# tencent-ailab/V-Express

Measured on AMD Instinct MI355X. Metric: decoded frames/sec at 512x512, 25 DDIM steps, higher is better.
Workload: dtype bf16; 1 GPU; 512x512, 16 frames (1 window(s) of 16, overlap 4), 25 DDIM steps, CFG 3.5, random-init UNet3D + ReferenceNet banks + sd-vae-ft-mse decode; frames=16, windows=1, parallelism=window x CFG-half units over 1 GPU(s)

## Files before the change

### v-express_amd/csrc/vx_attn.hip

```cpp
#include "vx_common.h"
#include <stdio.h>
#include "../../include/vexpress_hip.h"

#include <stdlib.h>

#include <type_traits>

namespace {

struct AttnParams {
  const bf16_t* q; int ldq;
  const bf16_t* k; int ldk;
  const bf16_t* vt; int vt_pitch;
  bf16_t* out; int ldo;
  int batch, heads, n_q, n_kv, d, q_per_kv;
  float c;
  const float* kmax;
};

__device__ __forceinline__ int k_lds_off(int slab, int key, int grp) {
  return slab * 4096 + key * 64 + ((grp ^ ((0 - (key >> 2)) & 3)) << 4);
}
__device__ __forceinline__ int v_lds_off(int row, int chunk) { return row * 128 + ((chunk ^ ((row >> 1) & 7)) << 4); }

// ... 658 lines not shown
    for (int half = 0; half < 2; ++half) {
      bf16_t e0 = 0, e1 = 0, e2 = 0, e3 = 0;
      if (half < FT && dcol < 32 * KK) {
        int fr0 = 16 * half + 4 * g;
        e0 = vsm[wave][fr0 + 0][dcol]; e1 = vsm[wave][fr0 + 1][dcol];
        e2 = vsm[wave][fr0 + 2][dcol]; e3 = vsm[wave][fr0 + 3][dcol];
      }
      w[2 * half + 0] = (uint32_t)e0 | ((uint32_t)e1 << 16);
      w[2 * half + 1] = (uint32_t)e2 | ((uint32_t)e3 << 16);
    }
    uint4 vf = make_uint4(w[0], w[1], w[2], w[3]);
#pragma unroll
    for (int qt = 0; qt < FT; ++qt) {
      f32x4_t acc = mfma16(vf, pb[qt], f32x4_t{0.f, 0.f, 0.f, 0.f});
      int fr = 16 * qt + i;
      int dc = 16 * dt + 4 * g;
      if (live && fr < p.f && dc < p.d) {
        uint2 st;
        st.x = pack_bf16x2(acc[0] * inv_l[qt], acc[1] * inv_l[qt]);
        st.y = pack_bf16x2(acc[2] * inv_l[qt], acc[3] * inv_l[qt]);
        *reinterpret_cast<uint2*>(p.out + ((size_t)(bb * p.f + fr) * p.hw + pix) * p.ldo + h * p.d + dc) = st;
      }
    }
  }
}

template <int KK, int DT>
int launch_temporal(const TemporalParams& p, hipStream_t stream) {
  long waves = (long)p.b * p.hw * p.heads;
  static int wpb_env = -1;
  if (wpb_env < 0) {
    const char* e = getenv("VX_TEMPORAL_WPB");
    wpb_env = e ? atoi(e) : 0;
  }
  const bool wide = wpb_env ? wpb_env == 8 : (p.heads % 8) == 0;
  static char sym[4][56];
  auto name = [&](int slot, int ft, int wpb) {
    if (!sym[slot][0]) snprintf(sym[slot], sizeof(sym[slot]), "temporal_attn_kernel<%d, %d, %d, %d>", KK, DT, ft, wpb);
    g_vx_last_kernel = sym[slot];
  };
  if (wide && (p.heads % 8) == 0 && KK * (p.f <= 16 ? 1 : 2) <= 6) {
    dim3 grid((unsigned)((waves + 7) / 8));
    name(p.f <= 16 ? 0 : 1, p.f <= 16 ? 1 : 2, 8);
    if (p.f <= 16) hipLaunchKernelGGL((temporal_attn_kernel<KK, DT, 1, 8>), grid, dim3(512), 0, stream, p);
    else hipLaunchKernelGGL((temporal_attn_kernel<KK, DT, 2, 8>), grid, dim3(512), 0, stream, p);
    return vx_check_launch("vx_temporal_attention");
  }
  dim3 grid((unsigned)((waves + 3) / 4));
  name(p.f <= 16 ? 2 : 3, p.f <= 16 ? 1 : 2, 4);
  if (p.f <= 16) hipLaunchKernelGGL((temporal_attn_kernel<KK, DT, 1, 4>), grid, dim3(256), 0, stream, p);
  else hipLaunchKernelGGL((temporal_attn_kernel<KK, DT, 2, 4>), grid, dim3(256), 0, stream, p);
  return vx_check_launch("vx_temporal_attention");
}

constexpr int SKV_MAX = 16;

__global__ __launch_bounds__(256) void small_kv_attn_kernel(const bf16_t* __restrict__ q, int ldq,
                                                            const bf16_t* __restrict__ kv, int ldkv, int v_off,
                                                            bf16_t* __restrict__ out, int ldo, int n_q, int n_kv,
                                                            int heads, int d, float c) {
  extern __shared__ __attribute__((aligned(16))) char smem[];
  bf16_t* kvs = reinterpret_cast<bf16_t*>(smem);
  const int C = heads * d;
  const int b = blockIdx.y;
  const int tid = threadIdx.x;
  const int cch = C >> 3;
  for (int idx = tid; idx < n_kv * 2 * cch; idx += 256) {
    int j = idx / (2 * cch), rem = idx % (2 * cch);
    int which = rem / cch, ch = (rem % cch) * 8;
    const bf16_t* src = kv + ((size_t)b * n_kv + j) * ldkv + (which ? v_off : 0) + ch;
    *reinterpret_cast<uint4*>(kvs + ((size_t)(j * 2 + which)) * C + ch) = *reinterpret_cast<const uint4*>(src);
  }
  __syncthreads();
  const long item = (long)blockIdx.x * 256 + tid;
  if (item >= (long)n_q * heads) return;
  const int h = (int)(item % heads);
  const int tok = (int)(item / heads);
  const bf16_t* qp = q + ((size_t)b * n_q + tok) * ldq + h * d;
  float sc[SKV_MAX];
#pragma unroll
  for (int j = 0; j < SKV_MAX; ++j) sc[j] = 0.f;
  for (int ch = 0; ch < d; ch += 8) {
    float qv[8];
    unpack_bf16x8(*reinterpret_cast<const uint4*>(qp + ch), qv);
#pragma unroll
    for (int j = 0; j < SKV_MAX; ++j) {
      if (j < n_kv) {
        float kvv[8];
        unpack_bf16x8(*reinterpret_cast<const uint4*>(kvs + (size_t)(j * 2) * C + h * d + ch), kvv);
#pragma unroll
        for (int e = 0; e < 8; ++e) sc[j] = fmaf(qv[e], kvv[e], sc[j]);
      }
    }
  }
  float mx = -INFINITY;
#pragma unroll
  for (int j = 0; j < SKV_MAX; ++j)
    if (j < n_kv) mx = fmaxf(mx, sc[j]);
  float den = 0.f;
#pragma unroll
  for (int j = 0; j < SKV_MAX; ++j) {
    float pv = (j < n_kv) ? __builtin_amdgcn_exp2f((sc[j] - mx) * c) : 0.f;
    sc[j] = pv;
    den += pv;
  }
  const float inv = 1.0f / den;
  bf16_t* op = out + ((size_t)b * n_q + tok) * ldo + h * d;
  for (int ch = 0; ch < d; ch += 8) {
    float acc[8] = {0.f, 0.f, 0.f, 0.f, 0.f, 0.f, 0.f, 0.f};
#pragma unroll
    for (int j = 0; j < SKV_MAX; ++j) {
      if (j < n_kv) {
        float vv[8];
        unpack_bf16x8(*reinterpret_cast<const uint4*>(kvs + (size_t)(j * 2 + 1) * C + h * d + ch), vv);
#pragma unroll
        for (int e = 0; e < 8; ++e) acc[e] = fmaf(sc[j], vv[e], acc[e]);
      }
    }
#pragma unroll
    for (int e = 0; e < 8; ++e) acc[e] *= inv;
    *reinterpret_cast<uint4*>(op + ch) = pack_bf16x8(acc);
  }
}

__global__ __launch_bounds__(256) void key_norm_max_kernel(const bf16_t* __restrict__ k, int ldk, int heads, int n_kv,
                                                           int d, float* __restrict__ out) {
  __shared__ float red[256];
  const int bh = blockIdx.x, b = bh / heads, h = bh - b * heads;
  const bf16_t* base = k + (size_t)b * n_kv * ldk + h * d;
  const int chunks = d >> 3;
  float best = 0.f;
  for (int key = threadIdx.x; key < n_kv; key += 256) {
    const bf16_t* row = base + (size_t)key * ldk;
    float ss = 0.f;
    for (int c = 0; c < chunks; ++c) {
      float f[8];
      unpack_bf16x8(*reinterpret_cast<const uint4*>(row + 8 * c), f);
#pragma unroll
      for (int e = 0; e < 8; ++e) ss = fmaf(f[e], f[e], ss);
    }
    best = fmaxf(best, ss);
  }
  red[threadIdx.x] = best;
  __syncthreads();
  for (int s = 128; s > 0; s >>= 1) {
    if ((int)threadIdx.x < s) red[threadIdx.x] = fmaxf(red[threadIdx.x], red[threadIdx.x + s]);
    __syncthreads();
  }
  if (threadIdx.x == 0) out[bh] = sqrtf(red[0]);
}

constexpr int KNM8_KEYS = 256;
__global__ __launch_bounds__(256) void key_norm_max8_kernel(const bf16_t* __restrict__ k, int ldk, int n_kv, int d,
                                                            float* __restrict__ out) {
  __shared__ float red[4][8];
  const int b = blockIdx.y, key0 = blockIdx.x * KNM8_KEYS;
  const int lane = threadIdx.x & 63, wave = threadIdx.x >> 6, h = lane & 7;
  const bf16_t* base = k + (size_t)b * n_kv * ldk + h * d;
  const int chunks = d >> 3;
  float best = 0.f;
  for (int kk = wave * 8 + (lane >> 3); kk < KNM8_KEYS; kk += 32) {
    const int key = min(key0 + kk, n_kv - 1);
    const bf16_t* row = base + (size_t)key * ldk;
    float ss = 0.f;
    for (int c = 0; c < chunks; ++c) {
      float f[8];
      unpack_bf16x8(*reinterpret_cast<const uint4*>(row + 8 * c), f);
#pragma unroll
      for (int e = 0; e < 8; ++e) ss = fmaf(f[e], f[e], ss);
    }
    best = fmaxf(best, ss);
  }
  best = fmaxf(best, __shfl_xor(best, 8, 64));
  best = fmaxf(best, __shfl_xor(best, 16, 64));
  best = fmaxf(best, __shfl_xor(best, 32, 64));
  if (lane < 8) red[wave][lane] = best;
  __syncthreads();
  if (threadIdx.x < 8) {
    const float m = fmaxf(fmaxf(red[0][threadIdx.x], red[1][threadIdx.x]), fmaxf(red[2][threadIdx.x], red[3][threadIdx.x]));
    atomicMax(reinterpret_cast<unsigned int*>(out) + b * 8 + threadIdx.x, __float_as_uint(sqrtf(m)));
  }
}

int attention_impl(const void* q, int ldq, const void* k, int ldk, const void* vt, int vt_pitch, void* out, int ldo,
                   int batch, int heads, int n_q, int n_kv, int head_dim, int q_per_kv, float scale,
                   const float* key_norm_max, hipStream_t stream);

}

int vx_attn3_variant();
int vx_attn3_launch(const void* q, int ldq, const void* k, int ldk, const void* vt, int vt_pitch, void* out, int ldo,
                    int batch, int heads, int n_q, int n_kv, int q_per_kv, float c, const float* kmax,
                    hipStream_t stream);

extern "C" int vx_key_norm_max(const void* k, int ldk, int kv_batches, int heads, int n_kv, int head_dim, float* out,
                               void* stream) {
  VX_REQUIRE(k && out, "vx_key_norm_max: null pointer");
  VX_REQUIRE(kv_batches > 0 && heads > 0 && n_kv > 0 && head_dim > 0 && (head_dim % 8) == 0 && (ldk % 8) == 0,
             "vx_key_norm_max: bad sizes (head_dim=%d ldk=%d)", head_dim, ldk);
  static int v8 = -1;
  if (v8 < 0) {
    const char* e = getenv("VX_KNM8");
    v8 = !(e && atoi(e) == 0);
  }
  if (v8 && heads == 8 && n_kv >= 2 * KNM8_KEYS && kv_batches <= 65535) {
    if (hipMemsetAsync(out, 0, (size_t)kv_batches * heads * sizeof(float), (hipStream_t)stream) != hipSuccess) {
      vx_set_error("vx_key_norm_max: hipMemsetAsync failed");
      return VX_ERR_HIP;
    }
    hipLaunchKernelGGL(key_norm_max8_kernel, dim3((n_kv + KNM8_KEYS - 1) / KNM8_KEYS, kv_batches), dim3(256), 0,
                       (hipStream_t)stream, (const bf16_t*)k, ldk, n_kv, head_dim, out);
    return vx_check_launch("vx_key_norm_max");
  }
  hipLaunchKernelGGL(key_norm_max_kernel, dim3(kv_batches * heads), dim3(256), 0, (hipStream_t)stream,
                     (const bf16_t*)k, ldk, heads, n_kv, head_dim, out);
  return vx_check_launch("vx_key_norm_max");
}

extern "C" int vx_attention(const void* q, int ldq, const void* k, int ldk, const void* vt, int vt_pitch, void* out,
                            int ldo, int batch, int heads, int n_q, int n_kv, int head_dim, int q_per_kv,
                            float scale, void* stream) {
  return attention_impl(q, ldq, k, ldk, vt, vt_pitch, out, ldo, batch, heads, n_q, n_kv, head_dim, q_per_kv, scale,
                        nullptr, (hipStream_t)stream);
}

extern "C" int vx_attention_bounded(const void* q, int ldq, const void* k, int ldk, const void* vt, int vt_pitch,
                                    void* out, int ldo, int batch, int heads, int n_q, int n_kv, int head_dim,
                                    int q_per_kv, float scale, const float* key_norm_max, void* stream) {
  VX_REQUIRE(key_norm_max != nullptr, "vx_attention_bounded: null key_norm_max");
  return attention_impl(q, ldq, k, ldk, vt, vt_pitch, out, ldo, batch, heads, n_q, n_kv, head_dim, q_per_kv, scale,
                        key_norm_max, (hipStream_t)stream);
}

namespace {
int attention_impl(const void* q, int ldq, const void* k, int ldk, const void* vt, int vt_pitch, void* out, int ldo,
                   int batch, int heads, int n_q, int n_kv, int head_dim, int q_per_kv, float scale,
                   const float* key_norm_max, hipStream_t stream) {
  VX_REQUIRE(q && k && vt && out, "vx_attention: null pointer");
  VX_REQUIRE(batch > 0 && heads > 0 && n_q > 0 && n_kv > 0 && q_per_kv > 0 && (batch % q_per_kv) == 0,
             "vx_attention: bad sizes");
  VX_REQUIRE((head_dim % 8) == 0 && (ldq % 8) == 0 && (ldk % 8) == 0 && (vt_pitch % 8) == 0 && (ldo % 4) == 0 &&
                 vt_pitch >= n_kv,
             "vx_attention: alignment (head_dim=%d ldq=%d ldk=%d pitch=%d ldo=%d)", head_dim, ldq, ldk, vt_pitch, ldo);
  VX_REQUIRE((long)batch * heads <= 65535, "vx_attention: batch*heads too large for grid.y");
  AttnParams p{(const bf16_t*)q, ldq, (const bf16_t*)k, ldk, (const bf16_t*)vt, vt_pitch, (bf16_t*)out, ldo,
               batch, heads, n_q, n_kv, head_dim, q_per_kv, scale == 0.f ? 1.0f : scale * 1.4426950408889634f,
               key_norm_max};
  VX_REQUIRE(scale >= 0.f, "vx_attention: scale must be positive (or 0: K carries scale * log2 e)");
  const int d = head_dim;
  static int v1 = -1;
  if (v1 < 0) v1 = getenv("VX_ATTN_V1") != nullptr;
  if (!v1 && d == 40 && key_norm_max && vx_attn3_variant() > 0 && ((size_t)n_kv * ldk * 2) < (1ull << 31) &&
      ((size_t)d * vt_pitch * 2) < (1ull << 31))
    return vx_attn3_launch(q, ldq, k, ldk, vt, vt_pitch, out, ldo, batch, heads, n_q, n_kv, q_per_kv, p.c, key_norm_max,
                           stream);
  if (!v1 && d > 32 && d <= 48 && (d % 16) != 0)
    return key_norm_max ? launch_attn2<2, 3, 2, true, true>(p, stream) : launch_attn2<2, 3, 2, true, false>(p, stream);
  if (d <= 32) return launch_attn<1, 2, 4, true>(p, stream);
  if (d <= 48) return launch_attn<2, 3, 2, true>(p, stream);
  if (d <= 64) return launch_attn<2, 4, 2, true>(p, stream);
  if (d <= 80) return launch_attn<3, 5, 2, true>(p, stream);
  if (d <= 96) return launch_attn<3, 6, 2, true>(p, stream);
  if (d <= 128) return launch_attn<4, 8, 2, true>(p, stream);
  if (d <= 160) return launch_attn<5, 10, 2, false>(p, stream);
  if (d == 512) return launch_attn<16, 32, 1, false, 1>(p, stream);
  vx_set_error("vx_attention: unsupported head_dim %d", d);
  return VX_ERR_UNSUPPORTED;
}
}

extern "C" int vx_temporal_attention(const void* qkv, int ldqkv, void* out, int ldo, int b, int f, int hw, int heads,
                                     int head_dim, float scale, void* stream_) {
  hipStream_t stream = (hipStream_t)stream_;
  VX_REQUIRE(qkv && out, "vx_temporal_attention: null pointer");
  VX_REQUIRE(f >= 1 && f <= 32, "vx_temporal_attention: f=%d outside [1,32] (PositionalEncoding max_len)", f);
  VX_REQUIRE((head_dim % 8) == 0 && (ldqkv % 8) == 0 && (ldo % 4) == 0, "vx_temporal_attention: alignment");
  TemporalParams p{(const bf16_t*)qkv, ldqkv, (bf16_t*)out, ldo, b, f, hw, heads, head_dim,
                   scale * 1.4426950408889634f};
  const int d = head_dim;
  if (d <= 32) return launch_temporal<1, 2>(p, stream);
  if (d <= 64) return launch_temporal<2, 4>(p, stream);
  if (d <= 96) return launch_temporal<3, 6>(p, stream);
  if (d <= 128) return launch_temporal<4, 8>(p, stream);
  if (d <= 160) return launch_temporal<5, 10>(p, stream);
  vx_set_error("vx_temporal_attention: unsupported head_dim %d", d);
  return VX_ERR_UNSUPPORTED;
}

extern "C" int vx_small_kv_attention(const void* q, int ldq, const void* kv, int ldkv, int v_off, void* out, int ldo,
                                     int batch, int n_q, int n_kv, int heads, int head_dim, float scale,
                                     void* stream_) {
  hipStream_t stream = (hipStream_t)stream_;
  VX_REQUIRE(q && kv && out, "vx_small_kv_attention: null pointer");
  VX_REQUIRE(n_kv >= 1 && n_kv <= SKV_MAX, "vx_small_kv_attention: n_kv=%d outside [1,%d]", n_kv, SKV_MAX);
  VX_REQUIRE((head_dim % 8) == 0 && (ldq % 8) == 0 && (ldkv % 8) == 0 && (v_off % 8) == 0 && (ldo % 8) == 0,
             "vx_small_kv_attention: alignment");
  const int C = heads * head_dim;
  size_t smem = (size_t)n_kv * 2 * C * sizeof(bf16_t);
  VX_REQUIRE(smem <= 64 * 1024, "vx_small_kv_attention: K/V tile %zu B exceeds LDS budget", smem);
  dim3 grid(ceil_div((long)n_q * heads, 256), batch);
  hipLaunchKernelGGL(small_kv_attn_kernel, grid, dim3(256), smem, stream, (const bf16_t*)q, ldq, (const bf16_t*)kv,
                     ldkv, v_off, (bf16_t*)out, ldo, n_q, n_kv, heads, head_dim, scale * 1.4426950408889634f);
  return vx_check_launch("vx_small_kv_attention");
}
```

### v-express_amd/ops.py

```python
import ctypes as C
import logging
import os

import torch

from . import lib as L

class _CurrentLib:

    def __getattr__(self, name):
        return getattr(L.current(), name)


_lib = _CurrentLib()


def __getattr__(name):
    if name == "BF16":
        return L.ELEM[0]
    raise AttributeError(name)


def _stream():
    return C.c_void_p(torch.cuda.current_stream().cuda_stream)
# ... 705 lines not shown
    p.wqkv_t, p.wo_t, p.colsum_p = (t.data_ptr() for t in hit[3:6])
    p.bias_o = bo.data_ptr() if bo is not None else None
    p.ln_stats = stats.data_ptr() if stats is not None else None
    p.stats_out = stats_out.data_ptr() if stats_out is not None else None
    p.ln_eps, p.scale = eps, (c // heads) ** -0.5
    with _hbm_op("tblock_fused", 2 * m * c * 2, flops=8.0 * m * c * c + 4.0 * m * f * c):
        L.check(_lib.vx_tblock_fused(C.byref(p), _stream()), "vx_tblock_fused")
    _set_gn(h)
    return h


def vt_pitch(n):
    return (n + 7) // 8 * 8


def gemm_split(a, w, bias, parts, *, part_cols, seq_len=0, head_dim=0, geom=None, ln=None):
    p, geom = _base_params(a, w, geom)
    p.epi = L.VX_EPI_SPLIT
    _set_ln(p, ln)
    p.bias = bias.data_ptr() if bias is not None else None
    p.part_cols, p.n_parts = part_cols, len(parts)
    p.seq_len, p.head_dim = seq_len, head_dim
    for i, (kind, t) in enumerate(parts):
        _chk_bf16(t, "part")
        p.part_out[i] = t.data_ptr()
        if kind == "rows":
            p.part_kind[i] = L.VX_PART_ROWS
            p.part_ld[i] = _row_stride(t)[0]
        else:
            p.part_kind[i] = L.VX_PART_VT
            p.part_ld[i] = 0
            p.vt_pitch = t.shape[-1]
            if not t.is_contiguous():
                raise ValueError("V^T destination must be contiguous")
    _launch_gemm(p, "vx_gemm(split)")


def alloc_vt(seqs, heads, head_dim, n, device):
    pitch = vt_pitch(n)
    if pitch != n:
        return torch.zeros((seqs, heads, head_dim, pitch), device=device, dtype=L.ELEM[0])
    return torch.empty((seqs, heads, head_dim, pitch), device=device, dtype=L.ELEM[0])


def _gn_slices(hw):
    return max(1, min(64, hw // 16))


_PADDED = {}


def padded_buffer(device, frames, H, W, c):
    key = (device, _stream_key(device), frames, H, W, c, L.ELEM[0])
    buf = _PADDED.get(key)
    if buf is None:
        buf = torch.zeros((frames, (H + 2) * (W + 2), c), device=device, dtype=L.ELEM[0])
        _PADDED[key] = buf
    return buf


def groupnorm(x1, gamma, beta, *, frames, hw, groups, eps, silu, x2=None, out=None, pad_hw=None):
    _chk_bf16(x1, "x1")
    if not x1.is_contiguous() or (x2 is not None and not x2.is_contiguous()):
        raise ValueError("groupnorm inputs must be contiguous")
    c1 = x1.shape[-1]
    c2 = x2.shape[-1] if x2 is not None else 0
    width, pad = hw, 0
    if pad_hw is not None:
        H, W = pad_hw
        if H * W != hw or out is not None:
            raise ValueError("pad_hw must factor hw and excludes `out`")
        out = padded_buffer(x1.device, frames, H, W, c1 + c2)
        width, pad = W, 1
    elif out is None:
        out = torch.empty((frames, hw, c1 + c2), device=x1.device, dtype=L.ELEM[0])
    slices = _gn_slices(hw)
    st = gn_of(x1) if x2 is None else None
    elems = frames * hw * (c1 + c2)
    if st is not None and st.fits(frames, hw, groups, c1):
        with _hbm_op("groupnorm_apply", 4 * elems):
            L.check(_lib.vx_groupnorm_apply(_ptr(x1), c1, None, 0, frames, hw, groups, float(eps), _ptr(gamma),
                                            _ptr(beta), int(silu), _ptr(out), _ptr(st.ws), st.slabs, slices, width, pad,
                                            _stream()), "vx_groupnorm_apply")
        return out
    ws = torch.empty(int(_lib.vx_groupnorm_ws_floats(frames, slices, groups)), device=x1.device,
                     dtype=torch.float32)
    with _hbm_op("groupnorm_stats+apply", 6 * elems):
        L.check(_lib.vx_groupnorm(_ptr(x1), c1, _ptr(x2), c2, frames, hw, groups, float(eps), _ptr(gamma), _ptr(beta),
                                  int(silu), _ptr(out), _ptr(ws), slices, width, pad, _stream()), "vx_groupnorm")
    return out


GN_FOLD = [os.environ.get("VX_GN_FOLD", "1") != "0" and os.environ.get("VX_GEMM_NOFAST") is None]


def gn_fold_applies(m, hw, c, n):
    items = _ITEMS[0]
    geom = (("c", c), ("n", n), ("hw", hw), ("rows_item", m // items if items and items > 0 and m % items == 0 else None))
    folded, applied = "GroupNorm folded into per-frame weights (no normalised tensor)", "GroupNorm apply pass + GEMM"
    if not GN_FOLD[0] or items is None or items <= 0 or m % items or hw % 256 or n % 320 or c % 64:
        return _note_path("groupnorm_proj_in", geom, False, applied, "fold off or geometry not whole 256 x 320 tiles per frame")
    if _ring_off(c):
        return _note_path("groupnorm_proj_in", geom, False, applied, "persistent kernel switched off")
    rows_item = m // items
    ok = rows_item % 256 == 0 and (2 * rows_item // 256) * (n // 320) >= 192 and n * 2 <= hw
    return _note_path("groupnorm_proj_in", geom, ok, folded if ok else applied,
                      "" if ok else "per-frame weight copies would cost more than the normalised tensor")


def groupnorm_stats(x1, *, frames, hw, groups, x2=None):
    _chk_bf16(x1, "x1")
    st = gn_of(x1) if x2 is None else None
    if st is not None and st.fits(frames, hw, groups, x1.shape[-1]):
        return st.ws, st.slabs
    if not x1.is_contiguous() or (x2 is not None and not x2.is_contiguous()):
        raise ValueError("groupnorm inputs must be contiguous")
    c1 = x1.shape[-1]
    c2 = x2.shape[-1] if x2 is not None else 0
    slices = _gn_slices(hw)
    ws = torch.empty(int(_lib.vx_groupnorm_ws_floats(frames, slices, groups)), device=x1.device, dtype=torch.float32)
    with _hbm_op("groupnorm_stats", 2 * frames * hw * (c1 + c2)):
        L.check(_lib.vx_groupnorm_stats(_ptr(x1), c1, _ptr(x2), c2, frames, hw, groups, _ptr(ws), slices, _stream()),
                "vx_groupnorm_stats")
    return ws, slices


def groupnorm_fold_linear(ws, gamma, w, bias_beta, *, frames, hw, groups, eps, slices=None):
    _chk_bf16(w, "w")
    n, c = w.shape
    if bias_beta.dtype != torch.float32 or gamma.dtype != torch.float32 or not w.is_contiguous():
        raise TypeError("groupnorm_fold_linear: float32 gamma / bias_beta, contiguous bf16 weight expected")
    w_f = torch.empty((frames, n, c), device=w.device, dtype=L.ELEM[0])
    b_f = torch.empty((frames, n), device=w.device, dtype=torch.float32)
    L.check(_lib.vx_groupnorm_fold_linear(_ptr(ws), frames, hw, slices or _gn_slices(hw), groups, float(eps), _ptr(gamma), c,
                                          _ptr(w), _ptr(bias_beta), n, _ptr(w_f), _ptr(b_f), _stream()),
            "vx_groupnorm_fold_linear")
    return w_f, b_f


def layernorm(x, gamma, beta, eps=1e-5, *, add=None, add_rows_per_entry=1, add_entries=1, out=None):
    _chk_bf16(x, "x")
    ldx, rows = _row_stride(x)
    c = x.shape[-1]
    if out is None:
        out = torch.empty((rows, c), device=x.device, dtype=L.ELEM[0])
    with _hbm_op("layernorm", 4 * rows * c):
        L.check(_lib.vx_layernorm(_ptr(x), ldx, rows, c, float(eps), _ptr(gamma), _ptr(beta), _ptr(add),
                                  add_rows_per_entry, add_entries, _ptr(out), _row_stride(out)[0], _stream()),
                "vx_layernorm")
    return out


_BOUNDED_SOFTMAX = [os.environ.get("VX_ATTN_BOUND", "1") != "0"]


def key_norm_max(k, *, kv_batches, heads, n_kv, head_dim):
    ldk, _ = _row_stride(k)
    out = torch.empty((kv_batches * heads,), device=k.device, dtype=torch.float32)
    with _hbm_op("key_norm_max", 2 * kv_batches * n_kv * heads * head_dim):
        L.check(_lib.vx_key_norm_max(_ptr(k), ldk, kv_batches, heads, n_kv, head_dim, _ptr(out), _stream()),
                "vx_key_norm_max")
    return out


def attention(q, k, vt, *, batch, heads, n_q, n_kv, head_dim, q_per_kv=1, out=None, kmax=None, k_prescaled=False):
    ldq, _ = _row_stride(q)
    ldk, _ = _row_stride(k)
    if out is None:
        out = torch.empty((batch * n_q, heads * head_dim), device=q.device, dtype=L.ELEM[0])
    scale = 0.0 if k_prescaled else head_dim ** -0.5
    c = heads * head_dim
    flops = 4.0 * batch * heads * n_q * n_kv * head_dim
    nbytes = 2 * (2 * batch * n_q * c + 2 * (batch // q_per_kv) * n_kv * c)
    if _BOUNDED_SOFTMAX[0] and 32 < head_dim <= 48 and head_dim % 16:
        if kmax is None:
            kmax = key_norm_max(k, kv_batches=batch // q_per_kv, heads=heads, n_kv=n_kv, head_dim=head_dim)
        with _hbm_op("attention", nbytes, flops=flops):
            L.check(_lib.vx_attention_bounded(_ptr(q), ldq, _ptr(k), ldk, _ptr(vt), vt.shape[-1], _ptr(out),
                                              _row_stride(out)[0], batch, heads, n_q, n_kv, head_dim, q_per_kv,
                                              scale, _ptr(kmax), _stream()), "vx_attention_bounded")
        return out
    with _hbm_op("attention", nbytes, flops=flops):
        L.check(_lib.vx_attention(_ptr(q), ldq, _ptr(k), ldk, _ptr(vt), vt.shape[-1], _ptr(out), _row_stride(out)[0],
                                  batch, heads, n_q, n_kv, head_dim, q_per_kv, scale, _stream()),
                "vx_attention")
    return out


def temporal_attention(qkv, *, b, f, hw, heads, head_dim, out=None):
    _chk_bf16(qkv, "qkv")
    ld, rows = _row_stride(qkv)
    if rows != b * f * hw:
        raise ValueError("qkv rows != b*f*hw")
    if out is None:
        out = torch.empty((rows, heads * head_dim), device=qkv.device, dtype=L.ELEM[0])
    with _hbm_op("temporal_attention", 2 * rows * 4 * heads * head_dim, flops=4.0 * rows * f * heads * head_dim):
        L.check(_lib.vx_temporal_attention(_ptr(qkv), ld, _ptr(out), _row_stride(out)[0], b, f, hw, heads, head_dim,
                                           head_dim ** -0.5, _stream()), "vx_temporal_attention")
    return out


def small_kv_attention(q, kv, *, batch, n_q, n_kv, heads, head_dim, out=None):
    ldq, _ = _row_stride(q)
    ldkv, _ = _row_stride(kv)
    c = heads * head_dim
    if out is None:
        out = torch.empty((batch * n_q, c), device=q.device, dtype=L.ELEM[0])
    with _hbm_op("small_kv_attention", 2 * (2 * batch * n_q * c + 2 * batch * n_kv * c)):
        L.check(_lib.vx_small_kv_attention(_ptr(q), ldq, _ptr(kv), ldkv, c, _ptr(out), _row_stride(out)[0], batch, n_q,
                                           n_kv, heads, head_dim, head_dim ** -0.5, _stream()),
                "vx_small_kv_attention")
    return out


UPSAMPLE_PHASES = [os.environ.get("VX_UPSAMPLE_PHASES", "1") != "0"]
UPSAMPLE_PHASES_MIN_HW = [int(os.environ.get("VX_UPSAMPLE_PHASES_MIN_HW", "256"))]


def upsample_phases_applies(H, W, c):
    geom = (("hw_in", H * W), ("c", c))
    four, one = "four 2x2 convolutions over the original image + interleave", "one 3x3 convolution with the upsampling in its gather"
    ok = UPSAMPLE_PHASES[0] and H * W >= UPSAMPLE_PHASES_MIN_HW[0] and c % 64 == 0
    return _note_path("upsample_conv", geom, ok, four if ok else one,
                      "" if ok else "switched off / input frame below VX_UPSAMPLE_PHASES_MIN_HW pixels / channels not a multiple of 64")


def pad_image(x, frames, H, W):
    _chk_bf16(x, "x")
    if not x.is_contiguous():
        raise ValueError("pad_image: contiguous input")
    c = x.shape[-1]
    out = padded_buffer(x.device, frames, H, W, c)
    L.check(_lib.vx_pad_image(_ptr(x), frames, H, W, c, _ptr(out), _stream()), "vx_pad_image")
    return out


def pixel_shuffle2x(phases, frames, H, W):
    _chk_bf16(phases, "phases")
    if phases.dim() != 3 or phases.shape[0] != 4 or phases.shape[1] != frames * H * W or not phases.is_contiguous():
        raise ValueError("pixel_shuffle2x: phases must be a contiguous [4, frames*H*W, C] tensor")
    c = phases.shape[-1]
    out = torch.empty((frames, 4 * H * W, c), device=phases.device, dtype=L.ELEM[0])
    L.check(_lib.vx_pixel_shuffle2x(_ptr(phases), phases.stride(0), frames, H, W, c, _ptr(out), _stream()), "vx_pixel_shuffle2x")
    return out


def upsample_conv_phases(x, w_phases, bias, *, frames, H, W):
    cout = w_phases.shape[1]
    xp = pad_image(x, frames, H, W)
    ph = torch.empty((4, frames * H * W, cout), device=x.device, dtype=L.ELEM[0])
    g = ConvGeom(frames, H + 2, W + 2, 2, 2, 1, 0, out_hw=(H, W))
    for a in (0, 1):
        for b in (0, 1):
            gemm(xp.view(frames * (H + 2) * (W + 2), -1), w_phases[a * 2 + b], bias, geom=g,
                 a_pixel_offset=a * (W + 2) + b, out=ph[a * 2 + b])
    return pixel_shuffle2x(ph, frames, H, W)


FF_PROJ_FOLD = [os.environ.get("VX_FF_PROJ_FOLD", "1") != "0"]
FF_PROJ_FOLD_MIN_HW = [int(os.environ.get("VX_FF_PROJ_FOLD_MIN_HW", "256"))]
FF_PROJ_FOLD_MM = [os.environ.get("VX_FF_PROJ_FOLD_MM", "1") != "0"]


def ff_proj_fold_applies(m, c, hidden):
    hw = _FRAME_ROWS[0]
    geom = (("c", c), ("hidden", hidden), ("hw", hw))
    one, two = "FF output GEMM + proj_out as one dual-source GEMM (K = 5C)", "two launches (FF output GEMM, proj_out)"
    if not FF_PROJ_FOLD[0] or FP8_PROJ[0]:
        return _note_path("ff_proj_out", geom, False, two, "switched off / fp8 projections")
    ok = hw is not None and hw >= FF_PROJ_FOLD_MIN_HW[0] and c % 64 == 0 and hidden % 64 == 0
    return _note_path("ff_proj_out", geom, ok, one if ok else two, "" if ok else "frame below VX_FF_PROJ_FOLD_MIN_HW rows")


AX_FUSED = [os.environ.get("VX_AX_FUSED", "1") != "0"]


class AudioFold:

    def __init__(self, kq, colsum, sbias, vo, frames, c):
        self.kq, self.colsum, self.sbias, self.vo, self.frames, self.c = kq, colsum, sbias, vo, frames, c


def audio_xattn_applies(c, heads, n_ctx, hw):
    geom = (("c", c), ("heads", heads), ("n_ctx", n_ctx), ("hw%16", hw % 16))
    one, three = "one launch (vx_audio_xattn)", "three launches (q GEMM + 5-key attention + output GEMM)"
    if not AX_FUSED[0] or not LN_FOLD[0] or FP8_PROJ[0]:
        return _note_path("audio_cross_attention", geom, False, three, "switched off / LayerNorm fold off / fp8 projections")
    ok = bool(_lib.vx_audio_xattn_supported(int(c), int(heads), int(n_ctx), int(hw)))
    return _note_path("audio_cross_attention", geom, ok, one if ok else three,
                      "" if ok else "the one-launch form is built for 8 heads, 5 audio tokens per frame, c % 320 == 0")


def audio_xattn_pack(kv, wq_folded, bq_folded, wo, *, frames, n_ctx, heads):
    _chk_bf16(kv, "kv")
    _chk_bf16(wq_folded, "wq")
    _chk_bf16(wo, "wo")
    c = wo.shape[0]
    if kv.shape != (frames * n_ctx, 2 * c) or tuple(wq_folded.shape) != (c, c) or tuple(wo.shape) != (c, c) or \
            not wq_folded.is_contiguous() or not wo.is_contiguous():
        raise ValueError("audio_xattn_pack: shapes")
    if bq_folded is not None and (bq_folded.dtype != torch.float32 or bq_folded.numel() != c):
        raise TypeError("audio_xattn_pack: folded bias must be float32 [C]")
    dev = kv.device
    kq = torch.empty((frames, 48 * c), device=dev, dtype=L.ELEM[0])
    vo = torch.empty((frames, 48 * c), device=dev, dtype=L.ELEM[0])
    cs = torch.empty((frames, 48), device=dev, dtype=torch.float32)
    sb = torch.empty((frames, 48), device=dev, dtype=torch.float32)
    L.check(_lib.vx_audio_xattn_pack(_ptr(kv), _row_stride(kv)[0], _ptr(wq_folded), _ptr(bq_folded), _ptr(wo), c, heads, n_ctx,
                                     frames, _ptr(kq), _ptr(cs), _ptr(sb), _ptr(vo), _stream()), "vx_audio_xattn_pack")
    return AudioFold(kq, cs, sb, vo, frames, c)


def audio_xattn(h, stats, fold, bias_o, alpha, *, rows_per_frame, stats_out=None, stats_eps=1e-5, out=None):
    _chk_bf16(h, "h")
    ldx, m = _row_stride(h)
    c = h.shape[-1]
    if out is None:
        out = h
    if m != fold.frames * rows_per_frame or c != fold.c:
        raise ValueError(f"audio_xattn: {m} rows of width {c} against operands for {fold.frames} frames x {rows_per_frame} rows, width {fold.c}")
    if stats.dtype != torch.float32 or not stats.is_contiguous() or tuple(stats.shape) not in ((m, 2), (m, 4)):
        raise ValueError("audio_xattn: stats must be a contiguous float32 [m, 2] / [m, 4] tensor")
    p = L.AxAttnParams()
    p.x, p.ldx, p.out, p.ldo = h.data_ptr(), ldx, out.data_ptr(), _row_stride(out)[0]
    p.rows, p.c, p.rows_per_frame = m, c, rows_per_frame
    p.ln_stats, p.ln_stats_parts, p.ln_eps = stats.data_ptr(), 2 if stats.shape[1] == 4 else 0, 1e-5
    p.kq, p.kq_colsum, p.kq_bias, p.vo = fold.kq.data_ptr(), fold.colsum.data_ptr(), fold.sbias.data_ptr(), fold.vo.data_ptr()
# ... 138 lines not shown
```

Baseline: 14.13 frames/s.

## Add bounded-softmax attention kernel for head dims 80 and 160

```diff
diff --git a/v-express_amd/csrc/vx_attn.hip b/v-express_amd/csrc/vx_attn.hip
--- a/v-express_amd/csrc/vx_attn.hip
+++ b/v-express_amd/csrc/vx_attn.hip
@@ -834,14 +834,14 @@
 
 constexpr int KNM8_KEYS = 256;
 __global__ __launch_bounds__(256) void key_norm_max8_kernel(const bf16_t* __restrict__ k, int ldk, int n_kv, int d,
-                                                            float* __restrict__ out) {
+                                                            int keys_per_block, float* __restrict__ out) {
   __shared__ float red[4][8];
-  const int b = blockIdx.y, key0 = blockIdx.x * KNM8_KEYS;
+  const int b = blockIdx.y, key0 = blockIdx.x * keys_per_block;
   const int lane = threadIdx.x & 63, wave = threadIdx.x >> 6, h = lane & 7;
   const bf16_t* base = k + (size_t)b * n_kv * ldk + h * d;
   const int chunks = d >> 3;
   float best = 0.f;
-  for (int kk = wave * 8 + (lane >> 3); kk < KNM8_KEYS; kk += 32) {
+  for (int kk = wave * 8 + (lane >> 3); kk < keys_per_block; kk += 32) {
     const int key = min(key0 + kk, n_kv - 1);
     const bf16_t* row = base + (size_t)key * ldk;
     float ss = 0.f;
@@ -874,6 +874,10 @@
 int vx_attn3_launch(const void* q, int ldq, const void* k, int ldk, const void* vt, int vt_pitch, void* out, int ldo,
                     int batch, int heads, int n_q, int n_kv, int q_per_kv, float c, const float* kmax,
                     hipStream_t stream);
+int vx_attn3d_variant();
+int vx_attn3d_launch(const void* q, int ldq, const void* k, int ldk, const void* vt, int vt_pitch, void* out, int ldo,
+                     int batch, int heads, int n_q, int n_kv, int head_dim, int q_per_kv, float c, const float* kmax,
+                     hipStream_t stream);
 
 extern "C" int vx_key_norm_max(const void* k, int ldk, int kv_batches, int heads, int n_kv, int head_dim, float* out,
                                void* stream) {
@@ -885,13 +889,15 @@
     const char* e = getenv("VX_KNM8");
     v8 = !(e && atoi(e) == 0);
   }
-  if (v8 && heads == 8 && n_kv >= 2 * KNM8_KEYS && kv_batches <= 65535) {
+  if (v8 && heads == 8 && n_kv >= 256 && kv_batches <= 65535) {
+    int kpb = KNM8_KEYS;
+    while (kpb > 32 && (long)kv_batches * ((n_kv + kpb - 1) / kpb) < 512) kpb >>= 1;
     if (hipMemsetAsync(out, 0, (size_t)kv_batches * heads * sizeof(float), (hipStream_t)stream) != hipSuccess) {
       vx_set_error("vx_key_norm_max: hipMemsetAsync failed");
       return VX_ERR_HIP;
     }
-    hipLaunchKernelGGL(key_norm_max8_kernel, dim3((n_kv + KNM8_KEYS - 1) / KNM8_KEYS, kv_batches), dim3(256), 0,
-                       (hipStream_t)stream, (const bf16_t*)k, ldk, n_kv, head_dim, out);
+    hipLaunchKernelGGL(key_norm_max8_kernel, dim3((n_kv + kpb - 1) / kpb, kv_batches), dim3(256), 0,
+                       (hipStream_t)stream, (const bf16_t*)k, ldk, n_kv, head_dim, kpb, out);
     return vx_check_launch("vx_key_norm_max");
   }
   hipLaunchKernelGGL(key_norm_max_kernel, dim3(kv_batches * heads), dim3(256), 0, (hipStream_t)stream,
@@ -932,10 +938,13 @@
   const int d = head_dim;
   static int v1 = -1;
   if (v1 < 0) v1 = getenv("VX_ATTN_V1") != nullptr;
-  if (!v1 && d == 40 && key_norm_max && vx_attn3_variant() > 0 && ((size_t)n_kv * ldk * 2) < (1ull << 31) &&
-      ((size_t)d * vt_pitch * 2) < (1ull << 31))
+  const bool dma_offsets_fit = ((size_t)n_kv * ldk * 2) < (1ull << 31) && ((size_t)d * vt_pitch * 2) < (1ull << 31);
+  if (!v1 && d == 40 && key_norm_max && vx_attn3_variant() > 0 && dma_offsets_fit)
     return vx_attn3_launch(q, ldq, k, ldk, vt, vt_pitch, out, ldo, batch, heads, n_q, n_kv, q_per_kv, p.c, key_norm_max,
                            stream);
+  if (!v1 && (d == 80 || d == 160) && key_norm_max && vx_attn3d_variant() > 0 && dma_offsets_fit)
+    return vx_attn3d_launch(q, ldq, k, ldk, vt, vt_pitch, out, ldo, batch, heads, n_q, n_kv, d, q_per_kv, p.c,
+                            key_norm_max, stream);
   if (!v1 && d > 32 && d <= 48 && (d % 16) != 0)
     return key_norm_max ? launch_attn2<2, 3, 2, true, true>(p, stream) : launch_attn2<2, 3, 2, true, false>(p, stream);
   if (d <= 32) return launch_attn<1, 2, 4, true>(p, stream);
diff --git a/v-express_amd/csrc/vx_attn3d.hip b/v-express_amd/csrc/vx_attn3d.hip
--- /dev/null
+++ b/v-express_amd/csrc/vx_attn3d.hip
@@ -0,0 +1,336 @@
+#include "vx_common.h"
+#include "vx_gemm_common.h"
+
+#include <stdlib.h>
+
+#include <type_traits>
+
+namespace {
+
+struct Attn3dParams {
+  const bf16_t* q; int ldq;
+  const bf16_t* k; int ldk;
+  const bf16_t* vt; int vt_pitch;
+  bf16_t* out; int ldo;
+  int batch, heads, n_q, n_kv, q_per_kv;
+  float c;
+  const float* kmax;
+};
+
+template <int D>
+struct A3dShape {
+  static constexpr int KK = (D + 31) / 32;
+  static constexpr int KFULL = D / 32;
+  static constexpr int KREM = (D % 32) / 8;
+  static constexpr int KBYTES = KFULL * 4096 + KREM * 1024;
+  static constexpr int VROWS = D + 16;
+  static constexpr int DT = VROWS / 16;
+  static constexpr int STAGE = KBYTES + VROWS * 128;
+  static constexpr int PIECES = KBYTES / 1024 + D / 8;
+  static constexpr int PPW = PIECES / 4;
+  static_assert(D % 16 == 0 && (KREM == 0 || KREM == 2) && PIECES % 4 == 0, "attn3d: unsupported head dim");
+};
+
+#ifdef VX_ATTN3D_COUNT
+__device__ unsigned int g_attn3d_count[2];
+#endif
+
+constexpr int A3D_QT = 2;
+
+__device__ __forceinline__ int a3d_pi(int r) { return 32 * (r >> 5) + 8 * ((r >> 2) & 3) + 4 * ((r >> 4) & 1) + (r & 3); }
+
+template <int D, int NBUF, bool UNIT>
+__global__ __launch_bounds__(256, D <= 80 ? 3 : 2) void attn3d_kernel(const Attn3dParams p) {
+  using S = A3dShape<D>;
+  constexpr int QT = A3D_QT, KK = S::KK, KFULL = S::KFULL, DT = S::DT, PPW = S::PPW;
+  static_assert(NBUF == 1 || NBUF == 2, "attn3d: one or two stages");
+  extern __shared__ __attribute__((aligned(16))) char smem[];
+  const int tid = threadIdx.x, lane = tid & 63;
+  const int wave = __builtin_amdgcn_readfirstlane(tid >> 6);
+  const int i = lane & 15, g = lane >> 4;
+  const int nqb = (p.n_q + 64 * QT - 1) / (64 * QT);
+  const int lid = xcd_remap(blockIdx.x, gridDim.x);
+  const int bh = lid / nqb, qb = lid - bh * nqb;
+  const int b = bh / p.heads, h = bh - b * p.heads;
+  const int kvb = b / p.q_per_kv;
+  const int q0 = qb * (64 * QT) + wave * (16 * QT);
+  const bf16_t* __restrict__ kbase = p.k + (size_t)kvb * p.n_kv * p.ldk + h * D;
+  const bf16_t* __restrict__ vbase = p.vt + (size_t)(kvb * p.heads + h) * D * p.vt_pitch;
+  const int n_tiles = (p.n_kv + 63) >> 6;
+  const bool ragged = (p.n_kv & 63) != 0;
+
+  for (int idx = tid; idx < NBUF * 128; idx += 256) {
+    const int st = idx >> 7, r = D + ((idx >> 3) & 15), j = idx & 7;
+    *reinterpret_cast<uint4*>(smem + st * S::STAGE + S::KBYTES + r * 128 + j * 16) =
+        r == D ? make_uint4(VX_E16_ONE2, VX_E16_ONE2, VX_E16_ONE2, VX_E16_ONE2) : make_uint4(0, 0, 0, 0);
+  }
+
+  uint32_t src0[PPW], src_edge[PPW];
+  const int te = n_tiles - 1;
+#pragma unroll
+  for (int s = 0; s < PPW; ++s) {
+    const int pw = wave + 4 * s;
+    if (pw < S::KBYTES / 1024) {
+      int r, chunk;
+      if (pw < 4 * KFULL) {
+        const int j = pw & 3;
+        r = 16 * j + (lane >> 2);
+        chunk = 4 * (pw >> 2) + ((lane & 3) ^ ((0 - (r >> 2)) & 3));
+      } else {
+        const int idx = 64 * (pw - 4 * KFULL) + lane;
+        r = idx >> 1;
+        chunk = 4 * KFULL + ((idx & 1) ^ ((r >> 3) & 1));
+      }
+      src0[s] = ((uint32_t)a3d_pi(r) * (uint32_t)p.ldk + 8u * chunk) * 2u;
+      uint32_t off = src0[s] + (uint32_t)te * 128u * (uint32_t)p.ldk;
+      const int over = te * 64 + a3d_pi(r) - (p.n_kv - 1);
+      if (over > 0) off -= (uint32_t)over * (uint32_t)p.ldk * 2u;
+      src_edge[s] = off;
+    } else {
+      const int j = pw - S::KBYTES / 1024;
+      const int r = 8 * j + (lane >> 3), chunk = (lane & 7) ^ ((r >> 1) & 7);
+      src0[s] = ((uint32_t)r * (uint32_t)p.vt_pitch + 8u * chunk) * 2u;
+      uint32_t off = src0[s] + (uint32_t)te * 128u;
+      if (te * 64 + 8 * chunk >= p.n_kv) off -= 16u * chunk;
+      src_edge[s] = off;
+    }
+  }
+  const uint32_t lds0 = lds_addr_of(smem);
+  const uint32_t kstep = 128u * (uint32_t)p.ldk;
+  auto issue = [&](int t) {
+    const uint32_t so = lds0 + (uint32_t)(t % NBUF) * S::STAGE;
+    const bool edge = ragged && t == n_tiles - 1;
+#pragma unroll
+    for (int s = 0; s < PPW; ++s) {
+      const int pw = wave + 4 * s;
+      const bool is_k = pw < S::KBYTES / 1024;
+      const uint32_t off = edge ? src_edge[s] : src0[s] + (uint32_t)t * (is_k ? kstep : 128u);
+      glds16_s(is_k ? (const void*)kbase : (const void*)vbase, off, so + pw * 1024);
+    }
+  };
+
+  uint4 qf[QT][KK];
+  float mfix[QT];
+#pragma unroll
+  for (int qt = 0; qt < QT; ++qt) {
+    const int qrow = q0 + 16 * qt + i;
+    float ss = 0.f;
+#pragma unroll
+    for (int kk = 0; kk < KK; ++kk) {
+      const int dcol = 32 * kk + 8 * g;
+      uint4 v = make_uint4(0, 0, 0, 0);
+      if (qrow < p.n_q && dcol < D) {
+        v = *reinterpret_cast<const uint4*>(p.q + (size_t)(b * p.n_q + qrow) * p.ldq + h * D + dcol);
+        float f[8];
+        unpack_bf16x8(v, f);
+#pragma unroll
+        for (int e = 0; e < 8; ++e) ss = fmaf(f[e], f[e], ss);
+      }
+      qf[qt][kk] = v;
+    }
+    ss = wave_xor_sum(ss, 16);
+    ss = wave_xor_sum(ss, 32);
+    mfix[qt] = sqrtf(ss) * p.kmax[kvb * p.heads + h] - (UNIT ? VX_P_HEADROOM : VX_P_HEADROOM / p.c);
+  }
+
+  const int a_k0 = i * 64 + ((g ^ ((0 - (i >> 2)) & 3)) << 4);
+  const int a_kp = KFULL * 4096 + i * 32 + (((g & 1) ^ ((i >> 3) & 1)) << 4);
+  const int vx = (i >> 1) & 7;
+  const int a_v0 = S::KBYTES + i * 128 + ((g ^ vx) << 4);
+  const int a_v1 = S::KBYTES + i * 128 + (((4 | g) ^ vx) << 4);
+
+  f32x4_t o[DT][QT];
+  auto zero_o = [&]() {
+#pragma unroll
+    for (int qt = 0; qt < QT; ++qt)
+#pragma unroll
+      for (int dt = 0; dt < DT; ++dt) o[dt][qt] = f32x4_t{0.f, 0.f, 0.f, 0.f};
+  };
+
+  auto qk = [&](f32x4_t (&s_)[4][QT], int t, const float (&m)[QT]) {
+    const char* kb = smem + (t % NBUF) * S::STAGE;
+#pragma unroll
+    for (int kt = 0; kt < 4; ++kt) {
+#pragma unroll
+      for (int qt = 0; qt < QT; ++qt) s_[kt][qt] = f32x4_t{-m[qt], -m[qt], -m[qt], -m[qt]};
+#pragma unroll
+      for (int kk = 0; kk < KK; ++kk) {
+        const uint4 kf = kk < KFULL ? *reinterpret_cast<const uint4*>(kb + a_k0 + kk * 4096 + kt * 1024)
+                                    : *reinterpret_cast<const uint4*>(kb + a_kp + kt * 512);
+#pragma unroll
+        for (int qt = 0; qt < QT; ++qt) s_[kt][qt] = mfma16(kf, qf[qt][kk], s_[kt][qt]);
+      }
+    }
+  };
+  auto mask = [&](f32x4_t (&s_)[4][QT], int t) {
+#pragma unroll
+    for (int kt = 0; kt < 4; ++kt)
+#pragma unroll
+      for (int r = 0; r < 4; ++r)
+        if (t * 64 + 32 * (kt >> 1) + 8 * g + 4 * (kt & 1) + r >= p.n_kv) {
+#pragma unroll
+          for (int qt = 0; qt < QT; ++qt) s_[kt][qt][r] = -INFINITY;
+        }
+  };
+  auto expo = [&](f32x4_t (&s_)[4][QT]) {
+#pragma unroll
+    for (int kt = 0; kt < 4; ++kt)
+#pragma unroll
+      for (int qt = 0; qt < QT; ++qt)
+#pragma unroll
+        for (int r = 0; r < 4; ++r) s_[kt][qt][r] = __builtin_amdgcn_exp2f(UNIT ? s_[kt][qt][r] : s_[kt][qt][r] * p.c);
+  };
+  auto pv = [&](const f32x4_t (&s_)[4][QT], int t) {
+    const int so = (t % NBUF) * S::STAGE;
+#pragma unroll
+    for (int ks_ = 0; ks_ < 2; ++ks_) {
+      uint4 pb[QT];
+#pragma unroll
+      for (int qt = 0; qt < QT; ++qt) {
+        const f32x4_t& a = s_[2 * ks_][qt];
+        const f32x4_t& c2 = s_[2 * ks_ + 1][qt];
+        pb[qt] = make_uint4(pack_bf16x2(a[0], a[1]), pack_bf16x2(a[2], a[3]), pack_bf16x2(c2[0], c2[1]),
+                            pack_bf16x2(c2[2], c2[3]));
+      }
+      const char* vp = smem + (ks_ ? a_v1 : a_v0) + so;
+#pragma unroll
+      for (int dt = 0; dt < DT; ++dt) {
+        const uint4 vf = *reinterpret_cast<const uint4*>(vp + dt * 2048);
+#pragma unroll
+        for (int qt = 0; qt < QT; ++qt) o[dt][qt] = mfma16(vf, pb[qt], o[dt][qt]);
+      }
+    }
+  };
+
+  float mrun[QT];
+  auto run = [&](auto maxpass_c, const float (&m)[QT]) {
+    constexpr bool MAXPASS = decltype(maxpass_c)::value;
+    __syncthreads();
+    issue(0);
+    for (int t = 0; t < n_tiles; ++t) {
+      if (NBUF == 1 && t > 0) {
+        __syncthreads();
+        issue(t);
+      }
+      asm volatile("s_waitcnt vmcnt(0)" ::: "memory");
+      __syncthreads();
+      if (NBUF == 2 && t + 1 < n_tiles) issue(t + 1);
+      f32x4_t cur[4][QT];
+      qk(cur, t, m);
+      if (ragged && t == n_tiles - 1) mask(cur, t);
+      if (MAXPASS) {
+#pragma unroll
+        for (int qt = 0; qt < QT; ++qt) {
+          float mx = mrun[qt];
+#pragma unroll
+          for (int kt = 0; kt < 4; ++kt)
+            mx = fmaxf(fmaxf(fmaxf(mx, cur[kt][qt][0]), fmaxf(cur[kt][qt][1], cur[kt][qt][2])), cur[kt][qt][3]);
+          mrun[qt] = mx;
+        }
+      } else {
+        expo(cur);
+        pv(cur, t);
+      }
+    }
+  };
+  auto row_sum = [&](int qt) -> float { return __shfl(o[DT - 1][qt][0], i, 64); };
+
+#ifdef VX_ATTN3D_COUNT
+  if (tid == 0) atomicAdd(&g_attn3d_count[0], 1u);
+#endif
+  zero_o();
+  run(std::false_type{}, mfix);
+  bool bad = false;
+#pragma unroll
+  for (int qt = 0; qt < QT; ++qt) {
+    const float l = row_sum(qt);
+    bad |= (q0 + 16 * qt + i < p.n_q) && !(l >= VX_P_MIN_ROWSUM(p.n_kv));
+  }
+  if (__syncthreads_or(bad)) {
+#ifdef VX_ATTN3D_COUNT
+    if (tid == 0) atomicAdd(&g_attn3d_count[1], 1u);
+#endif
+    const float zero[QT] = {0.f, 0.f};
+#pragma unroll
+    for (int qt = 0; qt < QT; ++qt) mrun[qt] = -INFINITY;
+    run(std::true_type{}, zero);
+#pragma unroll
+    for (int qt = 0; qt < QT; ++qt) mrun[qt] = wave_rows_max(mrun[qt]);
+    zero_o();
+    run(std::false_type{}, mrun);
+  }
+
+#pragma unroll
+  for (int qt = 0; qt < QT; ++qt) {
+    const float inv = 1.0f / row_sum(qt);
+    const int qrow = q0 + 16 * qt + i;
+    if (qrow >= p.n_q) continue;
+    bf16_t* orow = p.out + (size_t)(b * p.n_q + qrow) * p.ldo + h * D;
+#pragma unroll
+    for (int dt = 0; dt < D / 16; ++dt) {
+      uint2 w;
+      w.x = pack_bf16x2(o[dt][qt][0] * inv, o[dt][qt][1] * inv);
+      w.y = pack_bf16x2(o[dt][qt][2] * inv, o[dt][qt][3] * inv);
+      *reinterpret_cast<uint2*>(orow + 16 * dt + 4 * g) = w;
+    }
+  }
+}
+
+template <int D, int NBUF, bool UNIT>
+int launch_attn3d(const Attn3dParams& p, hipStream_t stream) {
+  constexpr int smem = NBUF * A3dShape<D>::STAGE;
+  auto kern = attn3d_kernel<D, NBUF, UNIT>;
+  static bool attr_set = false;
+  if (!attr_set) {
+    hipError_t e = hipFuncSetAttribute((const void*)kern, hipFuncAttributeMaxDynamicSharedMemorySize, smem);
+    if (e != hipSuccess) {
+      vx_set_error("vx_attention: hipFuncSetAttribute(%d) failed: %s", smem, hipGetErrorString(e));
+      return VX_ERR_HIP;
+    }
+    attr_set = true;
+  }
+  dim3 grid((unsigned)((long)ceil_div(p.n_q, 64 * A3D_QT) * p.batch * p.heads));
+  static char sym[64] = "";
+  if (!sym[0]) snprintf(sym, sizeof(sym), "attn3d_kernel<%d, %d, %s>", D, NBUF, UNIT ? "true" : "false");
+  g_vx_last_kernel = sym;
+  hipLaunchKernelGGL(kern, grid, dim3(256), smem, stream, p);
+  return vx_check_launch("vx_attention");
+}
+
+}
+
+int vx_attn3d_variant() {
+  static int v = -1;
+  if (v < 0) {
+    const char* e = getenv("VX_ATTN3D");
+    v = e ? atoi(e) : 1;
+  }
+  return v;
+}
+
+int vx_attn3d_launch(const void* q, int ldq, const void* k, int ldk, const void* vt, int vt_pitch, void* out, int ldo,
+                     int batch, int heads, int n_q, int n_kv, int head_dim, int q_per_kv, float c, const float* kmax,
+                     hipStream_t stream) {
+  Attn3dParams p{(const bf16_t*)q, ldq, (const bf16_t*)k, ldk, (const bf16_t*)vt, vt_pitch, (bf16_t*)out, ldo,
+                 batch, heads, n_q, n_kv, q_per_kv, c, kmax};
+  const bool unit = c == 1.0f;
+  if (head_dim == 80) return unit ? launch_attn3d<80, 2, true>(p, stream) : launch_attn3d<80, 2, false>(p, stream);
+  if (head_dim == 160) {
+    if (vx_attn3d_variant() == 2)
+      return unit ? launch_attn3d<160, 2, true>(p, stream) : launch_attn3d<160, 2, false>(p, stream);
+    return unit ? launch_attn3d<160, 1, true>(p, stream) : launch_attn3d<160, 1, false>(p, stream);
+  }
+  vx_set_error("vx_attention: attn3d has no head_dim %d", head_dim);
+  return VX_ERR_UNSUPPORTED;
+}
+
+#ifdef VX_ATTN3D_COUNT
+extern "C" int vx_attn3d_counts(unsigned int* counts, int reset) {
+  if (hipDeviceSynchronize() != hipSuccess ||
+      hipMemcpyFromSymbol(counts, HIP_SYMBOL(g_attn3d_count), 2 * sizeof(unsigned int)) != hipSuccess)
+    return VX_ERR_HIP;
+  const unsigned int zero[2] = {0u, 0u};
+  if (reset && hipMemcpyToSymbol(HIP_SYMBOL(g_attn3d_count), zero, sizeof(zero)) != hipSuccess) return VX_ERR_HIP;
+  return VX_OK;
+}
+#endif
diff --git a/v-express_amd/ops.py b/v-express_amd/ops.py
--- a/v-express_amd/ops.py
+++ b/v-express_amd/ops.py
@@ -881,6 +881,15 @@
 
 
 _BOUNDED_SOFTMAX = [os.environ.get("VX_ATTN_BOUND", "1") != "0"]
+_BOUNDED_WIDE_DIMS = [os.environ.get("VX_ATTN3D", "1") != "0" and os.environ.get("VX_ATTN_V1") is None]
+
+
+def _bounded_applies(head_dim, n_kv, have_table):
+    if not _BOUNDED_SOFTMAX[0]:
+        return False
+    if 32 < head_dim <= 48 and head_dim % 16:
+        return True
+    return _BOUNDED_WIDE_DIMS[0] and (head_dim == 80 or (head_dim == 160 and (have_table or n_kv >= 256)))
 
 
 def key_norm_max(k, *, kv_batches, heads, n_kv, head_dim):
@@ -901,7 +910,7 @@
     c = heads * head_dim
     flops = 4.0 * batch * heads * n_q * n_kv * head_dim
     nbytes = 2 * (2 * batch * n_q * c + 2 * (batch // q_per_kv) * n_kv * c)
-    if _BOUNDED_SOFTMAX[0] and 32 < head_dim <= 48 and head_dim % 16:
+    if _bounded_applies(head_dim, n_kv, kmax is not None):
         if kmax is None:
             kmax = key_norm_max(k, kv_batches=batch // q_per_kv, heads=heads, n_kv=n_kv, head_dim=head_dim)
         with _hbm_op("attention", nbytes, flops=flops):
```

Result: no change. 14.25 frames/s (median of 6 runs) (+0.9%).
